# joshua16266261/self-play-ai

Measured on AMD Instinct MI355X. Metric: MCTS sims/sec + self-play games/sec, Connect4 800 sims/move, 1/2/4/8 GPU, higher is better.
Workload: dtype bf16

## Files before the change

self-play-ai_amd/csrc/search.hip:

```cpp
#include <algorithm>
#include <cstdlib>
#include <cstring>

#include "search_internal.h"

namespace spai {
namespace {

constexpr int kLanesPerTree = 8;
#ifndef SPAI_TREE_BLOCK
#define SPAI_TREE_BLOCK 64
#endif
constexpr int kBlock = SPAI_TREE_BLOCK;
constexpr int kTreesPerBlock = kBlock / kLanesPerTree;
constexpr uint32_t kErrNan = 1u, kErrCapacity = 2u, kErrDepth = 4u;

constexpr uint32_t kPriorMark = 0x80000000u;
constexpr int kGenShift = 49;

__device__ __forceinline__ float ucb(float sqrt_np, const uint4 &ch, float c) {
    const uint32_t n = ch.x;
    const float w = __uint_as_float(ch.y), prior = __uint_as_float(ch.z);
    const float qv = ((-w / (float)(n == 0 ? 1u : n)) + 1.0f) / 2.0f;
    const float q = n == 0 ? 0.0f : qv;
    float u = c * prior;
    u = u * sqrt_np;
    u = u / (1.0f + (float)n);
    return q + u;
}

constexpr int kLevelsPerLane = kMaxDepth / kLanesPerTree;
__device__ __forceinline__ void backup_load(const uint4 *nodes, const uint32_t (&node)[kLevelsPerLane], int d,
                                            int lane8, uint2 (&r)[kLevelsPerLane]) {
#pragma unroll
    for (int j = 0; j < kLevelsPerLane; ++j) r[j] = *(const uint2 *)(nodes + (lane8 + 8 * j <= d ? node[j] : node[0]));
}
__device__ __forceinline__ void backup_store(uint4 *nodes, const uint32_t (&node)[kLevelsPerLane], int d, float v,
                                             int lane8, const uint2 (&r)[kLevelsPerLane]) {
#pragma unroll
    for (int j = 0; j < kLevelsPerLane; ++j) {
        const int lvl = lane8 + 8 * j;
        if (lvl <= d) {
            const float sign = ((d - lvl) & 1) ? -1.0f : 1.0f;
            *(uint2 *)(nodes + node[j]) = make_uint2(r[j].x + 1u, __float_as_uint(__uint_as_float(r[j].y) + sign * v));
        }
    }
}
__device__ __forceinline__ void backup_nodes(uint4 *nodes, const uint32_t (&node)[kLevelsPerLane], int d, float v,
                                             int lane8) {
    uint2 r[kLevelsPerLane];
    backup_load(nodes, node, d, lane8, r);
    backup_store(nodes, node, d, v, lane8, r);
}

__device__ __forceinline__ uint32_t group_bits(uint64_t ball) {
    return (uint32_t)(ball >> (threadIdx.x & 63 & ~(kLanesPerTree - 1))) & 0xFFu;
}

__device__ __forceinline__ bool has_line_flat(uint64_t b) {
    const uint64_t h = b & (b >> 7), v = b & (b >> 1), g = b & (b >> 8);
    return ((h & (h >> 14)) | (v & (v >> 2)) | (g & (g >> 16))) != 0ull;
}

__device__ __forceinline__ uint32_t score_key(float u) {
    const uint32_t b = __float_as_uint(u + 0.0f);
    return (b & 0x80000000u) ? ~b : (b | 0x80000000u);
}

struct Cand {
    uint32_t hi, lo, n, w;
};
template <int CTRL>
__device__ __forceinline__ uint32_t dpp_mov(uint32_t v) {
    return (uint32_t)__builtin_amdgcn_mov_dpp((int)v, CTRL, 0xF, 0xF, true);
}
template <int CTRL>
__device__ __forceinline__ void cand_step(Cand &c) {
    const Cand o{dpp_mov<CTRL>(c.hi), dpp_mov<CTRL>(c.lo), dpp_mov<CTRL>(c.n), dpp_mov<CTRL>(c.w)};
    const bool take = (((uint64_t)o.hi << 32) | o.lo) > (((uint64_t)c.hi << 32) | c.lo);
    c.hi = take ? o.hi : c.hi;
    c.lo = take ? o.lo : c.lo;
    c.n = take ? o.n : c.n;
    c.w = take ? o.w : c.w;
}

struct RootInfo {
    uint32_t node;
    uint64_t x, o;
    uint8_t n, status;
    uint32_t rn, rw;
};
__device__ __forceinline__ RootInfo load_root(const TreeView &T, uint32_t t) {
    const uint32_t node = T.root[t];
    const uint4 r = T.nodes[(size_t)t * T.cap + node];
    return RootInfo{node, T.root_x[t], T.root_o[t], T.root_n[t], T.root_status[t], r.x, r.w};
}

enum Descent { kTerminal = 0, kLive = 1, kError = 2 };
__device__ __forceinline__ Descent descend(const TreeView &T, uint32_t t, const RootInfo &root, int lane8, float c,
                                           uint32_t *err, uint64_t &x, uint64_t &o, uint8_t &n) {
    uint4 *nodes = T.nodes + (size_t)t * T.cap;
    uint32_t *path = T.path + (size_t)t * kMaxDepth;
    uint32_t node = root.node;
    x = root.x;
    o = root.o;
    n = root.n;
    uint8_t status = root.status;
    uint32_t rn = root.rn, rw = root.rw;
    uint32_t pr[kLevelsPerLane] = {node, 0u, 0u, 0u, 0u, 0u};
    const int top = 7 * lane8 + 5;
    int d = 0;
    if (lane8 == 0) path[0] = node;
    while (rw != kNoChildren) {
        const uint32_t first = rw & 0xFFFFFFu;
        const uint64_t occ = x | o;
        const bool open = lane8 < c4::kActions && !((occ >> top) & 1ull);
        const uint32_t k = c4::popc32(group_bits(__ballot(open)) & ((1u << lane8) - 1u));
        const uint4 ch = nodes[first + (open ? k : 0u)];
        const float sq = sqrtf((float)rn);
        const float u = ucb(sq, ch, c);
        Cand w{open ? score_key(u) : 0u, ((uint32_t)lane8 << 3) | k, ch.x, ch.w};
        cand_step<0xB1>(w);
        cand_step<0x4E>(w);
        cand_step<0x141>(w);
        if (group_bits(__ballot(open && u != u))) {
            if (lane8 == 0) atomicOr(err, kErrNan);
            return kError;
        }
        rn = w.n;
        rw = w.w;
        const int a = (int)(w.lo >> 3);
        const uint64_t bit = c4::drop_bit(occ, a);
        const bool xm = c4::x_to_move(n);
        x = xm ? x | bit : x;
        o = xm ? o : o | bit;
        n = (uint8_t)(n + 1);
        status = has_line_flat(xm ? x : o) ? c4::kWon : (n == c4::kCells ? c4::kTied : c4::kOngoing);
        node = first + (w.lo & 7u);
        ++d;
        if (d >= kMaxDepth) {
            if (lane8 == 0) atomicOr(err, kErrDepth);
            return kError;
        }
        const bool mine = (d & 7) == lane8;
        if (mine) path[d] = node;
#pragma unroll
        for (int j = 0; j < kLevelsPerLane; ++j) pr[j] = mine && (d >> 3) == j ? node : pr[j];
    }
    if (lane8 == 0) T.depth[t] = (uint8_t)d;
    if (status != c4::kOngoing) {
        backup_nodes(nodes, pr, d, c4::terminal_value(status), lane8);
        return kTerminal;
    }
    return kLive;
}

__device__ __forceinline__ uint4 *cache_way(const CacheView &C, uint64_t mine, uint64_t theirs, int way) {
    const uint64_t h = c4::splitmix64(mine ^ (theirs * 0x9E3779B97F4A7C15ull));
    const uint32_t bucket = (uint32_t)(h >> 32) & C.mask;
    return C.tab + ((size_t)bucket * EvalCache::kWays + (uint32_t)way) * 4;
}

__device__ __forceinline__ bool cache_insert(const CacheView &C, const BatchView &B, uint32_t s, int lane8) {
    const uint64_t mine = B.mine[s], theirs = B.theirs[s];
    const uint64_t gen = (uint64_t)C.gen << kGenShift;
    const uint64_t k0 = mine | gen, k1 = theirs | gen;
    uint4 *bucket = cache_way(C, mine, theirs, 0);
    const uint64_t seen = *(const uint64_t *)(bucket + 4 * lane8);
    const float4 pa = *(const float4 *)(B.priors + (size_t)s * kPriorStride);
    const float4 pb = *(const float4 *)(B.priors + (size_t)s * kPriorStride + 4);
    const float value = B.value[s];
    const uint32_t same = group_bits(__ballot(seen == k0));
    const uint32_t empty = group_bits(__ballot(seen == 0ull));
    if (same || lane8 != 0) return false;
    const uint32_t p0 = __float_as_uint(pa.x), p2 = __float_as_uint(pa.z), p4 = __float_as_uint(pb.x),
                   p6 = __float_as_uint(pb.z);
    bool claimed = false, skip = ((p0 | p2 | p4 | p6) & kPriorMark) != 0u;
    if (!skip)
        for (int w = empty ? __ffs(empty) - 1 : (int)EvalCache::kWays; w < (int)EvalCache::kWays; ++w) {
            uint4 *e = bucket + 4 * w;
            const unsigned long long old = atomicCAS((unsigned long long *)e, 0ull, (unsigned long long)k0);
            if (old == 0ull) {
                ((uint64_t *)e)[1] = k1;
                e[1] = make_uint4(p0 | kPriorMark, __float_as_uint(pa.y), p2 | kPriorMark, __float_as_uint(pa.w));
                e[2] = make_uint4(p4 | kPriorMark, __float_as_uint(pb.y), p6 | kPriorMark, __float_as_uint(value));
                claimed = true;
                break;
            }
            if (old == k0) {
                skip = true;
                break;
            }
        }
    if (!claimed && !skip) atomicAdd(C.ctr + 1, 1u);
    return claimed;
}
__device__ __forceinline__ void cache_count(const CacheView &C, bool claimed) {
    const uint64_t b = __ballot(claimed);
    if (b && (threadIdx.x & 63) == (uint32_t)__ffsll((unsigned long long)__ballot(true)) - 1u)
        atomicAdd(C.ctr, (uint32_t)c4::popc64(b));
}

__device__ __forceinline__ void slot_leaf(const TreeView &T, const BatchView &B, const CacheView &C, uint32_t t,
                                          int lane8, uint64_t x, uint64_t o, uint8_t n) {
    const bool xm = c4::x_to_move(n);
    const uint64_t mine = xm ? x : o, theirs = xm ? o : x;
    if (lane8 == 0)
        __hip_atomic_fetch_add(T.evals + t, 1u, __ATOMIC_RELAXED, __HIP_MEMORY_SCOPE_AGENT);
    if (C.tab) {
        const uint4 *e = cache_way(C, mine, theirs, lane8);
        const uint4 q0 = e[0], q1 = e[1], q2 = e[2];
        const uint64_t gen = (uint64_t)C.gen << kGenShift;
        const bool match = (((uint64_t)q0.y << 32) | q0.x) == (mine | gen) &&
                           (((uint64_t)q0.w << 32) | q0.z) == (theirs | gen) &&
                           (q1.x & q1.z & q2.x & q2.z & kPriorMark) != 0u;
        const uint32_t hit = group_bits(__ballot(match));
        if (hit) {
            uint32_t slot = 0;
            if (lane8 == 0) {
                slot = B.cap - 1u - atomicAdd(B.hits, 1u);
                T.slot[t] = slot | kHitSlot;
                B.tree[slot] = t;
                B.mine[slot] = mine;
                B.theirs[slot] = theirs;
            }
            slot = (uint32_t)__shfl((int)slot, 0, kLanesPerTree);
            if (lane8 == __ffs(hit) - 1) {
                float4 *pr = (float4 *)(B.priors + (size_t)slot * kPriorStride);
                pr[0] = make_float4(__uint_as_float(q1.x & ~kPriorMark), __uint_as_float(q1.y),
                                    __uint_as_float(q1.z & ~kPriorMark), __uint_as_float(q1.w));
                pr[1] = make_float4(__uint_as_float(q2.x & ~kPriorMark), __uint_as_float(q2.y),
                                    __uint_as_float(q2.z & ~kPriorMark), 0.f);
                B.value[slot] = __uint_as_float(q2.w);
            }
            return;
        }
    }
    if (lane8 == 0) {
        const uint32_t slot = atomicAdd(B.count, 1u);
        T.slot[t] = slot;
        B.tree[slot] = t;
        B.mine[slot] = mine;
        B.theirs[slot] = theirs;
    }
}

template <bool RUN_ON>
__device__ __forceinline__ void select_tree(const TreeView &T, const BatchView &B, const CacheView &C, uint32_t t,
                                            RootInfo &root, int lane8, float c, uint32_t *err, uint32_t run_cap) {
    if (lane8 == 0) T.slot[t] = kNoSlot;
    uint64_t x, o;
    uint8_t n;
    if (!RUN_ON) {
        if (descend(T, t, root, lane8, c, err, x, o, n) == kLive) slot_leaf(T, B, C, t, lane8, x, o, n);
        return;
    }
    uint32_t left = T.left[t];
    for (uint32_t run = 0; left > 0; ++run) {
        if (run == run_cap) {
            if (lane8 == 0) atomicOr(B.more, 1u);
            break;
        }
        --left;
        const Descent r = descend(T, t, root, lane8, c, err, x, o, n);
        if (r == kLive) slot_leaf(T, B, C, t, lane8, x, o, n);
        if (r != kTerminal) break;
        root.rn += 1;
        __builtin_amdgcn_fence(__ATOMIC_SEQ_CST, "wavefront");
    }
    if (lane8 == 0) T.left[t] = left;
}

struct LeafPath {
    int d;
    uint32_t lv[kLevelsPerLane];
    uint32_t first;
};
__device__ __forceinline__ LeafPath load_leaf_path(const TreeView &T, uint32_t t, int lane8) {
    LeafPath L;
    const uint32_t *path = T.path + (size_t)t * kMaxDepth;
    L.d = T.depth[t];
#pragma unroll
    for (int j = 0; j < kLevelsPerLane; ++j) L.lv[j] = path[lane8 + 8 * j];
    L.first = T.next_free[t];
    return L;
}

__device__ __forceinline__ void expand_leaf(const TreeView &T, const BatchView &B, uint32_t t, uint32_t s, int lane8,
                                            uint32_t *err, const LeafPath &L, RootInfo &root) {
    uint4 *nodes = T.nodes + (size_t)t * T.cap;
    const int d = L.d;
    uint32_t node[kLevelsPerLane];
#pragma unroll
    for (int j = 0; j < kLevelsPerLane; ++j) node[j] = lane8 + 8 * j <= d ? L.lv[j] : 0u;
    const uint64_t occ = B.mine[s] | B.theirs[s];
    const float prior = B.priors[(size_t)s * kPriorStride + lane8];
    const float value = B.value[s];
    uint2 r[kLevelsPerLane];
    backup_load(nodes, node, d, lane8, r);
    const bool legal = lane8 < c4::kActions && !((occ >> (7 * lane8 + 5)) & 1ull);
    const uint32_t grp = group_bits(__ballot(legal));
    const uint32_t nch = c4::popc32(grp);
    const uint32_t idx = c4::popc32(grp & ((1u << lane8) - 1u));
    const uint32_t first = L.first;
    if (first + nch > T.cap) {
        if (lane8 == 0) atomicOr(err, kErrCapacity);
        return;
    }
    if (legal) nodes[first + idx] = make_uint4(0u, 0u, __float_as_uint(prior), kNoChildren);
    if (lane8 == 0) T.next_free[t] = first + nch;
    if (lane8 == (d & 7)) {
        uint32_t leaf = node[0];
#pragma unroll
        for (int j = 1; j < kLevelsPerLane; ++j) leaf = (d >> 3) == j ? node[j] : leaf;
        nodes[leaf].w = first | (nch << 24);
    }
    backup_store(nodes, node, d, value, lane8, r);
    root.rn += 1;
    if (d == 0) root.rw = first | (nch << 24);
}

template <bool RUN_ON>
__global__ __launch_bounds__(kBlock) void k_select(TreeView T, BatchView B, CacheView C,
                                                   const uint32_t *__restrict__ active, uint32_t n_active, float c,
                                                   uint32_t *err, uint32_t run_cap) {
    const uint32_t gi = (blockIdx.x * blockDim.x + threadIdx.x) / kLanesPerTree;
#ifdef SPAI_TREE_PRIO
    __builtin_amdgcn_s_setprio(SPAI_TREE_PRIO);
#endif
    if (gi >= n_active) return;
    const uint32_t t = active[gi];
    RootInfo root = load_root(T, t);
    select_tree<RUN_ON>(T, B, C, t, root, threadIdx.x & (kLanesPerTree - 1), c, err, run_cap);
}

template <bool RUN_ON>
__global__ __launch_bounds__(kBlock) void k_expand_select(TreeView T, BatchView cur, BatchView nxt, CacheView C,
                                                          const uint32_t *__restrict__ active, uint32_t n_active,
                                                          float c, uint32_t *err, uint32_t run_cap) {
    const uint32_t gi = (blockIdx.x * blockDim.x + threadIdx.x) / kLanesPerTree;
#ifdef SPAI_TREE_PRIO
    __builtin_amdgcn_s_setprio(SPAI_TREE_PRIO);
#endif
    if (gi >= n_active) return;
    const int lane8 = threadIdx.x & (kLanesPerTree - 1);
    const uint32_t t = active[gi];
    const uint32_t s = T.slot[t];
    RootInfo root = load_root(T, t);
    const LeafPath L = load_leaf_path(T, t, lane8);
    asm volatile("" ::"v"(root.rn), "v"(root.rw), "v"((uint32_t)root.x), "v"((uint32_t)(root.x >> 32)),
                 "v"((uint32_t)root.o), "v"((uint32_t)(root.o >> 32)), "v"((uint32_t)root.n), "v"((uint32_t)root.status));
    asm volatile("" ::"v"(L.d), "v"(L.first), "v"(L.lv[0]), "v"(L.lv[1]), "v"(L.lv[2]), "v"(L.lv[3]), "v"(L.lv[4]),
                 "v"(L.lv[5]));
    if (s != kNoSlot) expand_leaf(T, cur, t, s & ~kHitSlot, lane8, err, L, root);
    __builtin_amdgcn_fence(__ATOMIC_SEQ_CST, "wavefront");
    select_tree<RUN_ON>(T, nxt, C, t, root, lane8, c, err, run_cap);
    if (C.tab) {
        const bool claimed = s != kNoSlot && !(s & kHitSlot) && cache_insert(C, cur, s, lane8);
        cache_count(C, claimed);
    }
}

__global__ void k_set_left(TreeView T, const uint32_t *__restrict__ active, uint32_t n, uint32_t iters) {
    const uint32_t i = blockIdx.x * blockDim.x + threadIdx.x;
    if (i < n) T.left[active[i]] = iters;
}

__global__ __launch_bounds__(kBlock) void k_eval_stub(BatchView B, uint32_t max_n, int kind) {
    const uint32_t s = blockIdx.x * blockDim.x + threadIdx.x;
    if (s >= max_n || s >= *B.count) return;
    const uint32_t n = (uint32_t)c4::popc64(B.mine[s] | B.theirs[s]);
    const bool xm = (n & 1u) == 0;
    const uint64_t x = xm ? B.mine[s] : B.theirs[s], o = xm ? B.theirs[s] : B.mine[s];
    float pr[c4::kActions], v;
    c4::stub_eval(kind, x, o, (uint8_t)n, pr, &v);
    for (int a = 0; a < c4::kActions; ++a) B.priors[(size_t)s * kPriorStride + a] = pr[a];
    B.value[s] = v;
}

__global__ __launch_bounds__(kBlock) void k_expand(TreeView T, BatchView B, CacheView C, uint32_t max_n,
                                                   uint32_t *err) {
    const uint32_t i = (blockIdx.x * blockDim.x + threadIdx.x) / kLanesPerTree;
    if (i >= max_n) return;
    const uint32_t count = *B.count, hits = B.hits ? *B.hits : 0u;
    if (i >= count + hits) return;
    const bool fwd = i < count;
    const uint32_t s = fwd ? i : B.cap - 1u - (i - count);
    const int lane8 = threadIdx.x & (kLanesPerTree - 1);
    const uint32_t t = B.tree[s];
    RootInfo root{};
    expand_leaf(T, B, t, s, lane8, err, load_leaf_path(T, t, lane8), root);
    if (C.tab) {
        const bool claimed = fwd && cache_insert(C, B, s, lane8);
        cache_count(C, claimed);
    }
}

__global__ void k_root_stats(TreeView T, const uint32_t *__restrict__ active, uint32_t n_active, uint32_t *out,
                             uint32_t *max_evals) {
    const uint32_t i = blockIdx.x * blockDim.x + threadIdx.x;
    if (i >= n_active) return;
    const uint32_t t = active[i];
    atomicMax(max_evals, T.evals[t]);
    atomicAdd(max_evals + 1, T.evals[t]);
    const uint4 *nodes = T.nodes + (size_t)t * T.cap;
    const uint4 r = nodes[T.root[t]];
    out[i * 8] = r.w;
    const uint32_t nch = r.w == kNoChildren ? 0 : r.w >> 24, first = r.w & 0xFFFFFFu;
    for (uint32_t k = 0; k < 7; ++k) out[i * 8 + 1 + k] = k < nch ? nodes[first + k].x : 0u;
}

__global__ void k_trees_init(TreeView T, RootsOut R, uint32_t first_tree, uint32_t n) {
    const uint32_t i = blockIdx.x * blockDim.x + threadIdx.x;
    if (i < n) tree_clear(T, R, first_tree + i);
}
}

TreeView tree_view(spai_engine *e) {
    Trees &T = e->trees;
    return TreeView{T.nodes.p, T.cap, T.root.p, T.next_free.p, T.root_x.p, T.root_o.p, T.root_n.p, T.root_status.p,
                    T.path.p, T.depth.p, T.slot.p, T.left.p, T.evals.p};
}

static BatchView batch_view(spai_engine *e, int chain, uint32_t it, bool cached) {
    Batch &B = e->batch[chain];
    const size_t h = (size_t)(it & 1u) * B.cap;
    return BatchView{B.iter_counts.p + it, B.iter_more.p ? B.iter_more.p + it : nullptr, B.tree.p + h, B.mine.p + h, B.theirs.p + h,
                     B.priors.p + h * kPriorStride, B.value.p + h,
                     cached ? B.iter_hits.p + it : nullptr, B.cap};
}

CacheView cache_view(spai_engine *e) {
    EvalCache &C = e->cache;
    if (!C.buckets) return CacheView{nullptr, 0u, 0u, nullptr};
    return CacheView{C.table.p, C.buckets - 1u, C.gen, C.ctr.p};
}

int cache_clear(spai_engine *e) {
    EvalCache &C = e->cache;
    if (!C.buckets) return SPAI_OK;
    uint32_t fill = 0;
    SPAI_HIP(hipMemcpyAsync(&fill, C.ctr.p, 4, hipMemcpyDeviceToHost, e->stream));
    SPAI_HIP(hipStreamSynchronize(e->stream));
    C.inserts_cleared += fill;
    SPAI_HIP(hipMemsetAsync(C.table.p, 0, C.table.n * sizeof(uint4), e->stream));
    SPAI_HIP(hipMemsetAsync(C.ctr.p, 0, 4, e->stream));
    C.gen = C.gen % 32767u + 1u;
    C.fill_seen = 0;
    C.clears += 1;
    return SPAI_OK;
}

int cache_prepare(spai_engine *e, bool for_net) {
    EvalCache &C = e->cache;
    if (C.ready && C.for_net == for_net) return SPAI_OK;
    C.for_net = for_net;
    uint64_t want = 0;
    if (for_net) {
        const char *v = std::getenv("SPAI_EVAL_CACHE");
        if (C.user_set) want = C.requested;
        else if (v) want = std::strtoull(v, nullptr, 10);
        else want = std::min<uint64_t>(EvalCache::kEntriesPerTree * std::max(1u, e->cfg.max_trees),
                                       EvalCache::kDefaultMaxEntries);
    }
    uint32_t buckets = 0;
    if (want) {
        buckets = 1;
        while ((uint64_t)buckets * 2 * EvalCache::kWays <= want && buckets < (1u << 28)) buckets *= 2;
    }
    if (buckets != C.buckets) {
        SPAI_HIP(hipStreamSynchronize(e->stream));
        if (C.buckets) {
            uint32_t fill = 0;
            SPAI_HIP(hipMemcpy(&fill, C.ctr.p, 4, hipMemcpyDeviceToHost));
            C.inserts_cleared += fill;
        }
        C.buckets = 0;
        if (C.ctr.p) SPAI_HIP(hipMemsetAsync(C.ctr.p, 0, 4, e->stream));
        const bool by_default = !C.user_set && !std::getenv("SPAI_EVAL_CACHE");
        int rc = C.table.alloc((size_t)buckets * EvalCache::kWays * 4);
        while (rc != SPAI_OK && by_default) {
            (void)hipGetLastError();
            buckets = buckets / 2 >= EvalCache::kMinDefaultBuckets ? buckets / 2 : 0;
            rc = C.table.alloc((size_t)buckets * EvalCache::kWays * 4);
        }
        SPAI_TRY(rc);
        if (buckets) {
            if (!C.ctr.p) {
                SPAI_TRY(C.ctr.alloc(2));
                SPAI_HIP(hipMemsetAsync(C.ctr.p, 0, 8, e->stream));
            }
            C.buckets = buckets;
            SPAI_TRY(cache_clear(e));
        }
    }
    C.ready = true;
    return SPAI_OK;
}

constexpr double kMinChainLeaves = 64;
constexpr double kTailLeaves = 0.05;
constexpr uint32_t kTailTreeEvals = 160;
constexpr uint32_t kTailRun = 128;
static int env_int(const char *name, int dflt) {
    const char *v = std::getenv(name);
    return v ? std::atoi(v) : dflt;
}
struct ChainPolicy {
    int chains;
    uint32_t grid_cap;
};
static ChainPolicy chains_for(uint32_t n, double last_evals_per_iter) {
    static const int forced = std::max(0, std::min(spai_engine::kChains, env_int("SPAI_CHAINS", 0)));
    static const int mid_leaves = env_int("SPAI_MID_LEAVES", 0);
    static const int mid_chains = std::max(1, std::min(spai_engine::kChains, env_int("SPAI_MID_CHAINS", 2)));
    static const uint32_t mid_grid = (uint32_t)std::max(0, env_int("SPAI_MID_GRID", 0));
    static const double min_chain_leaves = env_int("SPAI_MIN_CHAIN_LEAVES", (int)kMinChainLeaves);
    static const int hi_leaves = env_int("SPAI_HI_LEAVES", 0);
    if (forced) return {std::max(1, std::min<int>(forced, (int)(n / 64))), 0u};
    if (hi_leaves > 0 && (last_evals_per_iter < 0 ? (double)n : last_evals_per_iter) >= hi_leaves) return {1, 0u};
    if (last_evals_per_iter >= 0 && last_evals_per_iter < min_chain_leaves) return {1, 0u};
    if (last_evals_per_iter >= 0 && last_evals_per_iter < mid_leaves)
        return {std::max(1, std::min<int>(mid_chains, (int)(n / 64))), mid_grid};
    return {std::max(1, std::min<int>(2, (int)(n / 64))), 0u};
}

static int upload_roots(spai_engine *e, uint32_t t0, uint32_t n) {
    Trees &T = e->trees;
    std::vector<uint64_t> x(n), o(n);
    std::vector<uint8_t> nn(n), st(n);
    for (uint32_t i = 0; i < n; ++i) {
        const c4::State &s = T.h_root_state[t0 + i];
        x[i] = s.x;
        o[i] = s.o;
        nn[i] = s.n;
        st[i] = s.status;
    }
    hipStream_t s = e->stream;
    SPAI_HIP(hipMemcpyAsync(T.root.p + t0, T.h_root.data() + t0, n * 4, hipMemcpyHostToDevice, s));
    SPAI_HIP(hipMemcpyAsync(T.root_x.p + t0, x.data(), n * 8, hipMemcpyHostToDevice, s));
    SPAI_HIP(hipMemcpyAsync(T.root_o.p + t0, o.data(), n * 8, hipMemcpyHostToDevice, s));
    SPAI_HIP(hipMemcpyAsync(T.root_n.p + t0, nn.data(), n, hipMemcpyHostToDevice, s));
    SPAI_HIP(hipMemcpyAsync(T.root_status.p + t0, st.data(), n, hipMemcpyHostToDevice, s));
    SPAI_HIP(hipStreamSynchronize(s));
    return SPAI_OK;
}

static int timer_record(spai_engine *e, int which, uint32_t iter, bool begin, hipStream_t st, int chain) {
    KernelTimer &K = e->timer;
    if (!K.enabled) return SPAI_OK;
    if (begin) {
        if (K.used + 2 > K.ev.size()) {
            for (int i = 0; i < 64; ++i) {
                hipEvent_t ev;
                SPAI_HIP(hipEventCreate(&ev));
                K.ev.push_back(ev);
            }
        }
        K.which.push_back(which);
        K.iter.push_back(iter);
        K.chain.push_back(chain);
        SPAI_HIP(hipEventRecord(K.ev[K.used], st));
    } else {
        SPAI_HIP(hipEventRecord(K.ev[K.used + 1], st));
        K.used += 2;
    }
    return SPAI_OK;
}

static int timer_collect(spai_engine *e, const uint32_t *ch_counts, uint32_t num_searches, const Chain *chains) {
    KernelTimer &K = e->timer;
    if (!K.enabled) return SPAI_OK;
    for (size_t i = 0; i < K.which.size(); ++i) {
        float ms = 0;
        SPAI_HIP(hipEventElapsedTime(&ms, K.ev[2 * i], K.ev[2 * i + 1]));
        const int w = K.which[i], h = K.chain[i];
        K.total_ms[w] += ms;
        K.launches[w] += 1;
        K.items[w] += w == 0 ? chains[h].cnt : ch_counts[(size_t)h * num_searches + K.iter[i]];
    }
    K.used = 0;
    K.which.clear();
    K.iter.clear();
    K.chain.clear();
    return SPAI_OK;
}

int trees_create(spai_engine *e, uint32_t n) {
    SPAI_CHECK(n > 0 && n <= e->cfg.max_trees, SPAI_ERR_INVALID, "trees_create: n=%u exceeds max_trees=%u", n,
               e->cfg.max_trees);
    Trees &T = e->trees;
    const uint64_t cap = 1ull + (uint64_t)c4::kActions * e->cfg.num_searches * std::max(1u, e->cfg.max_moves);
    SPAI_CHECK(cap < (1ull << 24), SPAI_ERR_CAPACITY, "node arena of %llu nodes per tree exceeds 2^24",
               (unsigned long long)cap);
    if (T.n_trees != n || T.cap != cap) {
        T.n_trees = 0;
        SPAI_TRY(T.nodes.alloc((size_t)n * cap));
        SPAI_TRY(T.root.alloc(n));
        SPAI_TRY(T.next_free.alloc(n));
        SPAI_TRY(T.root_x.alloc(n));
        SPAI_TRY(T.root_o.alloc(n));
        SPAI_TRY(T.root_n.alloc(n));
        SPAI_TRY(T.root_status.alloc(n));
        SPAI_TRY(T.path.alloc((size_t)n * kMaxDepth));
        SPAI_TRY(T.depth.alloc(n));
        SPAI_TRY(T.slot.alloc(n));
        SPAI_TRY(T.left.alloc(n));
        SPAI_TRY(T.evals.alloc(n + 2));
        SPAI_TRY(T.slot_gid.alloc(n));
        SPAI_TRY(T.slot_move.alloc(n));
        SPAI_TRY(T.refill.alloc(2 * (size_t)n));
        SPAI_TRY(e->active.alloc(n));
        SPAI_TRY(e->stats.alloc((size_t)n * 8));
        for (Batch &B : e->batch) {
            SPAI_TRY(B.tree.alloc(2 * (size_t)n));
            SPAI_TRY(B.mine.alloc(2 * (size_t)n));
            SPAI_TRY(B.theirs.alloc(2 * (size_t)n));
            SPAI_TRY(B.priors.alloc(2 * (size_t)n * kPriorStride));
            SPAI_TRY(B.value.alloc(2 * (size_t)n));
            B.cap = n;
        }
        T.n_trees = n;
        T.cap = (uint32_t)cap;
    }
    e->last_evals_per_iter = -1;
    e->last_served_per_iter = -1;
    e->last_max_tree_evals = ~0u;
    T.h_root.assign(n, 0);
    T.h_root_state.assign(n, c4::State{0, 0, 0, c4::kOngoing});
    T.h_root_first.assign(n, 0);
    T.h_root_nch.assign(n, 0);
    k_trees_init<<<(n + 255) / 256, 256, 0, e->stream>>>(tree_view(e), roots_out(e), 0, n);
    SPAI_HIP(hipGetLastError());
    return upload_roots(e, 0, n);
}

int tree_reset(spai_engine *e, uint32_t t, const spai_c4_state *root) {
    Trees &T = e->trees;
    SPAI_CHECK(t < T.n_trees, SPAI_ERR_INVALID, "tree %u out of range", t);
    c4::State s{0, 0, 0, c4::kOngoing};
    if (root) {
        SPAI_CHECK(!(root->x & root->o) && !((root->x | root->o) & ~c4::kBoard) && root->status <= c4::kWon,
                   SPAI_ERR_INVALID, "root is not a Connect4 bitboard");
        s = from_abi(*root);
    }
    T.h_root[t] = 0;
    T.h_root_state[t] = s;
    T.h_root_first[t] = 0;
    T.h_root_nch[t] = 0;
    k_trees_init<<<1, 64, 0, e->stream>>>(tree_view(e), roots_out(e), t, 1);
    SPAI_HIP(hipGetLastError());
    return upload_roots(e, t, 1);
}

static int evaluate(const Chain &c, hipStream_t st, const BatchView &bv, uint32_t grid_cap, int conc) {
    if (c.kind == SPAI_EVAL_NET)
        return net_eval_batch(c.net, st, bv.count, c.cnt, bv.mine, bv.theirs, bv.priors, bv.value, grid_cap, conc);
    k_eval_stub<<<(c.cnt + kBlock - 1) / kBlock, kBlock, 0, st>>>(bv, c.cnt, c.kind);
    return SPAI_OK;
}

int chains_launch(spai_engine *e, const uint32_t *trees, const Chain *chains, int nchain, uint32_t grid_cap, bool timed,
                  bool tail) {
    hipStream_t st = e->stream;
    uint32_t n = 0, iters = 0;
    int conc = 0;
    for (int h = 0; h < nchain; ++h) {
        const Chain &c = chains[h];
        if (!c.cnt) continue;
        n += c.cnt;
        iters = std::max(iters, c.iters);
        conc += c.kind == SPAI_EVAL_NET;
        Batch &B = e->batch[h];
        const uint32_t nc = std::max<uint32_t>(c.iters, 1) + (tail ? kTailChunk + 1 : 0);
        DevBuf<uint32_t> *ctr[3] = {&B.iter_counts, c.cache.tab ? &B.iter_hits : nullptr,
                                    tail ? &B.iter_more : nullptr};
        for (DevBuf<uint32_t> *b : ctr) {
            if (!b) continue;
            if (b->n < nc) SPAI_TRY(b->alloc(nc));
            SPAI_HIP(hipMemsetAsync(b->p, 0, (size_t)nc * 4, st));
        }
    }
    SPAI_HIP(hipMemcpyAsync(e->active.p, trees, (size_t)n * 4, hipMemcpyHostToDevice, st));
    SPAI_HIP(hipMemsetAsync(e->err.p, 0, 4, st));
    SPAI_HIP(hipMemsetAsync(e->trees.evals.p, 0, ((size_t)e->trees.n_trees + 2) * 4, st));
    if (n > chains[0].cnt) SPAI_HIP(hipEventRecord(e->ev_fork, st));
    for (int h = 1; h < nchain; ++h)
        if (chains[h].cnt) SPAI_HIP(hipStreamWaitEvent(e->chain_stream[h], e->ev_fork, 0));
    const TreeView tv = tree_view(e);
    timed = timed && e->timer.enabled;
    for (uint32_t it = 0; it < (tail ? 0u : iters); ++it) {
        for (int h = 0; h < nchain; ++h) {
            const Chain &c = chains[h];
            if (!c.cnt || it >= c.iters) continue;
            const hipStream_t sh = e->chain_stream[h];
            const BatchView bv = batch_view(e, h, it, c.cache.tab);
            const uint32_t nh = c.cnt, g8 = (nh + kTreesPerBlock - 1) / kTreesPerBlock;
            const uint32_t *act = e->active.p + c.off;
            const bool sample = timed && (it % e->timer.stride == 0);
            if (it == 0) {
                if (sample) SPAI_TRY(timer_record(e, 0, it, true, sh, h));
                k_select<false><<<g8, kBlock, 0, sh>>>(tv, bv, c.cache, act, nh, e->cfg.c, e->err.p, 0u);
                if (sample) SPAI_TRY(timer_record(e, 0, it, false, sh, h));
            }
            if (sample) SPAI_TRY(timer_record(e, 1, it, true, sh, h));
            SPAI_TRY(evaluate(c, sh, bv, grid_cap, std::max(conc, 1)));
            if (sample) SPAI_TRY(timer_record(e, 1, it, false, sh, h));
            if (it + 1 < c.iters) {
                const bool s2 = timed && ((it + 1) % e->timer.stride == 0);
                if (s2) SPAI_TRY(timer_record(e, 0, it + 1, true, sh, h));
                k_expand_select<false><<<g8, kBlock, 0, sh>>>(tv, bv, batch_view(e, h, it + 1, c.cache.tab), c.cache,
                                                              act, nh, e->cfg.c, e->err.p, 0u);
                if (s2) SPAI_TRY(timer_record(e, 0, it + 1, false, sh, h));
            } else {
                if (sample) SPAI_TRY(timer_record(e, 2, it, true, sh, h));
                k_expand<<<g8, kBlock, 0, sh>>>(tv, bv, c.cache, nh, e->err.p);
                if (sample) SPAI_TRY(timer_record(e, 2, it, false, sh, h));
            }
        }
    }
    SPAI_HIP(hipGetLastError());
    for (int h = 1; h < nchain; ++h) {
        if (!chains[h].cnt) continue;
        SPAI_HIP(hipEventRecord(e->ev_join[h], e->chain_stream[h]));
        SPAI_HIP(hipStreamWaitEvent(st, e->ev_join[h], 0));
    }
    return SPAI_OK;
}

int search_launch(spai_engine *e, uint32_t n, const uint32_t *tree_idx, uint32_t num_searches, SearchRun &R) {
    const int kind = (int)e->cfg.eval;
    hipStream_t st = e->stream;
    SPAI_TRY(cache_prepare(e, kind == SPAI_EVAL_NET));
    if (cache_nearly_full(e->cache)) SPAI_TRY(cache_clear(e));
    const char *tl_env = std::getenv("SPAI_TAIL_LEAVES");
    const char *tt_env = std::getenv("SPAI_TAIL_TREE_EVALS");
    const double tail_leaves = tl_env ? std::atof(tl_env) : kTailLeaves;
    const uint32_t tail_tree = tt_env ? (uint32_t)std::max(0, std::atoi(tt_env)) : kTailTreeEvals;
    const bool tail = num_searches > 0 && e->last_served_per_iter >= 0 &&
                      (e->last_served_per_iter < tail_leaves || e->last_max_tree_evals < tail_tree);
    const bool solved = e->last_served_per_iter == 0.0;
    const char *tr_env = std::getenv("SPAI_TAIL_RUN");
    const uint32_t tail_run =
        tr_env ? (uint32_t)std::max(1, std::atoi(tr_env)) : (solved ? std::max(num_searches, 1u) : kTailRun);
    const uint32_t tail_chunk = solved ? 1u : kTailChunk;
    const ChainPolicy pol = tail ? ChainPolicy{1, 0u} : chains_for(n, e->last_evals_per_iter);
    const int nchain = R.nchain = pol.chains;
    const CacheView cv = cache_view(e);
    for (int h = 0; h < nchain; ++h) {
        const uint32_t off = (uint32_t)((uint64_t)n * h / nchain);
        R.chain[h] = Chain{off, (uint32_t)((uint64_t)n * (h + 1) / nchain) - off, num_searches, kind, e->net, cv};
    }
    SPAI_TRY(chains_launch(e, tree_idx, R.chain, nchain, pol.grid_cap, true, tail));
    R.n_counts = num_searches;
    if (tail) {
        const TreeView tv = tree_view(e);
        const uint32_t g8 = (n + kTreesPerBlock - 1) / kTreesPerBlock;
        const uint32_t *act = e->active.p;
        k_set_left<<<(n + 255) / 256, 256, 0, st>>>(tv, act, n, num_searches);
        k_select<true><<<g8, kBlock, 0, st>>>(tv, batch_view(e, 0, 0, cv.tab), cv, act, n, e->cfg.c, e->err.p, tail_run);
        uint32_t p = 0, next = 1, more = 0, next_hits = 0;
        for (;;) {
            for (uint32_t q = 0; q < tail_chunk; ++q, ++p) {
                const BatchView bv = batch_view(e, 0, p, cv.tab);
                SPAI_TRY(evaluate(R.chain[0], st, bv, 0u, 1));
                k_expand_select<true><<<g8, kBlock, 0, st>>>(tv, bv, batch_view(e, 0, p + 1, cv.tab), cv, act, n,
                                                             e->cfg.c, e->err.p, tail_run);
            }
            SPAI_HIP(hipGetLastError());
            SPAI_HIP(hipMemcpyAsync(&next, e->batch[0].iter_counts.p + p, 4, hipMemcpyDeviceToHost, st));
            SPAI_HIP(hipMemcpyAsync(&more, e->batch[0].iter_more.p + p, 4, hipMemcpyDeviceToHost, st));
            if (cv.tab)
                SPAI_HIP(hipMemcpyAsync(&next_hits, e->batch[0].iter_hits.p + p, 4, hipMemcpyDeviceToHost, st));
            SPAI_HIP(hipStreamSynchronize(st));
            next += next_hits;
            if (next == 0 && more == 0) break;
            SPAI_CHECK(p <= num_searches + 1, SPAI_ERR_INVALID, "internal: tail passes exceed the iterations");
        }
        R.n_counts = p;
    }
    e->last_tail_passes = tail ? R.n_counts : 0;
    return SPAI_OK;
}

int check_device_errors(spai_engine *e, uint32_t err) {
    SPAI_CHECK(!(err & kErrCapacity), SPAI_ERR_CAPACITY, "node arena full (cap %u per tree)", e->trees.cap);
    SPAI_CHECK(!(err & kErrDepth), SPAI_ERR_CAPACITY, "tree deeper than %d", kMaxDepth);
    SPAI_CHECK(!(err & kErrNan), SPAI_ERR_NAN, "NaN UCB in select (reference: partial_cmp().unwrap() panics)");
    return SPAI_OK;
}

void cache_account(spai_engine *e, double served, double forwarded, uint32_t fill) {
    if (!e->cache.buckets) return;
    e->cache.lookups += served;
    e->cache.hits += served - forwarded;
    e->cache.fill_seen = fill;
}

int search_finish(spai_engine *e, const SearchRun &R, uint32_t num_searches, const uint32_t *ch_counts, uint32_t err,
                  uint32_t max_tree_evals, double served, uint32_t cache_fill) {
    SPAI_TRY(timer_collect(e, ch_counts, R.n_counts, R.chain));
    double s = 0;
    for (int h = 0; h < R.nchain; ++h)
        for (uint32_t i = 0; i < R.n_counts; ++i) s += ch_counts[(size_t)h * R.n_counts + i];
    SPAI_TRY(check_device_errors(e, err));
    cache_account(e, served, s, cache_fill);
    e->last_evals_per_iter = num_searches ? s / num_searches : -1;
    e->last_served_per_iter = num_searches ? served / num_searches : -1;
    e->last_max_tree_evals = max_tree_evals;
    return SPAI_OK;
}

int search(spai_engine *e, uint32_t n, const uint32_t *tree_idx, uint32_t num_searches, float *policy,
           uint32_t *child_ids, float *child_visits, uint32_t *n_children, double *evals_out) {
    Trees &T = e->trees;
    SPAI_CHECK(T.n_trees > 0, SPAI_ERR_INVALID, "no trees: call spai_trees_create first");
    SPAI_CHECK(n <= T.n_trees, SPAI_ERR_INVALID, "search over %u trees, %u exist", n, T.n_trees);
    for (uint32_t i = 0; i < n; ++i) SPAI_CHECK(tree_idx[i] < T.n_trees, SPAI_ERR_INVALID, "tree %u out of range", tree_idx[i]);
    const int kind = (int)e->cfg.eval;
    SPAI_CHECK(kind != SPAI_EVAL_NET || e->net, SPAI_ERR_INVALID, "eval = NET but no net set (spai_engine_set_net)");
    if (n == 0) return SPAI_OK;
    hipStream_t st = e->stream;
    SearchRun R;
    SPAI_TRY(search_launch(e, n, tree_idx, num_searches, R));
    const TreeView tv = tree_view(e);
    const int nchain = R.nchain;
    const uint32_t n_counts = R.n_counts;
    k_root_stats<<<(n + 255) / 256, 256, 0, st>>>(tv, e->active.p, n, e->stats.p, T.evals.p + T.n_trees);
    SPAI_HIP(hipGetLastError());
    std::vector<uint32_t> stats((size_t)n * 8), ch_counts((size_t)nchain * n_counts);
    uint32_t err = 0, tree_evals[2] = {0, 0}, cache_fill = 0;
    SPAI_HIP(hipMemcpyAsync(stats.data(), e->stats.p, stats.size() * 4, hipMemcpyDeviceToHost, st));
    SPAI_HIP(hipMemcpyAsync(tree_evals, T.evals.p + T.n_trees, 8, hipMemcpyDeviceToHost, st));
    if (e->cache.buckets) SPAI_HIP(hipMemcpyAsync(&cache_fill, e->cache.ctr.p, 4, hipMemcpyDeviceToHost, st));
    if (n_counts)
        for (int h = 0; h < nchain; ++h)
            SPAI_HIP(hipMemcpyAsync(ch_counts.data() + (size_t)h * n_counts, e->batch[h].iter_counts.p,
                                    n_counts * 4, hipMemcpyDeviceToHost, st));
    SPAI_HIP(hipMemcpyAsync(&err, e->err.p, 4, hipMemcpyDeviceToHost, st));
    SPAI_HIP(hipStreamSynchronize(st));
    SPAI_TRY(search_finish(e, R, num_searches, ch_counts.data(), err, tree_evals[0], tree_evals[1], cache_fill));
    if (evals_out) *evals_out = (double)tree_evals[1];
    for (uint32_t i = 0; i < n; ++i) {
        const uint32_t t = tree_idx[i];
        const uint32_t w = stats[i * 8];
        const uint32_t nch = w == kNoChildren ? 0 : w >> 24, first = w & 0xFFFFFFu;
        T.h_root_first[t] = first;
        T.h_root_nch[t] = (uint8_t)nch;
        const c4::State &rs = T.h_root_state[t];
        const uint32_t legal = c4::legal_mask(rs.x, rs.o, rs.status);
        float pol[c4::kActions] = {0, 0, 0, 0, 0, 0, 0};
        for (uint32_t k = 0; k < nch; ++k) {
            const float v = (float)stats[i * 8 + 1 + k];
            pol[c4::kth_bit(legal, (int)k)] = v;
            if (child_ids) child_ids[(size_t)i * 7 + k] = first + k;
            if (child_visits) child_visits[(size_t)i * 7 + k] = v;
        }
        for (uint32_t k = nch; k < 7; ++k) {
            if (child_ids) child_ids[(size_t)i * 7 + k] = kNoChildren;
            if (child_visits) child_visits[(size_t)i * 7 + k] = 0.f;
        }
        if (n_children) n_children[i] = nch;
        if (policy) normalize_policy(pol, policy + (size_t)i * 7);
    }
    return SPAI_OK;
}

int tree_use_subtree(spai_engine *e, uint32_t t, uint32_t child) {
    Trees &T = e->trees;
    SPAI_CHECK(t < T.n_trees, SPAI_ERR_INVALID, "tree %u out of range", t);
    const uint32_t first = T.h_root_first[t], nch = T.h_root_nch[t];
    SPAI_CHECK(nch > 0 && child >= first && child < first + nch, SPAI_ERR_INVALID,
               "node %u is not a child of tree %u's root (run spai_search first)", child, t);
    const c4::State &rs = T.h_root_state[t];
    c4::State ns;
    const int a = c4::kth_bit(c4::legal_mask(rs.x, rs.o, rs.status), (int)(child - first));
    SPAI_CHECK(c4::next_state(rs, a, ns) == 0, SPAI_ERR_INVALID, "internal: root child replay failed");
    T.h_root[t] = child;
    T.h_root_state[t] = ns;
    T.h_root_nch[t] = 0;
    return upload_roots(e, t, 1);
}

int tree_node(spai_engine *e, uint32_t t, uint32_t node, spai_c4_state *st, uint32_t *visits, float *w) {
    Trees &T = e->trees;
    SPAI_CHECK(t < T.n_trees, SPAI_ERR_INVALID, "tree %u out of range", t);
    c4::State s = T.h_root_state[t];
    if (node != T.h_root[t]) {
        const uint32_t first = T.h_root_first[t], nch = T.h_root_nch[t];
        SPAI_CHECK(nch > 0 && node >= first && node < first + nch, SPAI_ERR_INVALID,
                   "node %u: only the root and its children are addressable", node);
        const int a = c4::kth_bit(c4::legal_mask(s.x, s.o, s.status), (int)(node - first));
        c4::State ns;
        c4::next_state(s, a, ns);
        s = ns;
    }
    if (st) *st = to_abi(s);
    if (visits || w) {
        uint4 rec;
        SPAI_HIP(hipMemcpy(&rec, T.nodes.p + (size_t)t * T.cap + node, 16, hipMemcpyDeviceToHost));
        if (visits) *visits = rec.x;
        if (w) memcpy(w, &rec.y, 4);
    }
    return SPAI_OK;
}

int tree_size(spai_engine *e, uint32_t t, uint32_t *nodes) {
    Trees &T = e->trees;
    SPAI_CHECK(t < T.n_trees, SPAI_ERR_INVALID, "tree %u out of range", t);
    SPAI_HIP(hipMemcpy(nodes, T.next_free.p + t, 4, hipMemcpyDeviceToHost));
    return SPAI_OK;
}


int eval_cache_set_capacity(spai_engine *e, uint64_t entries) {
    e->cache.user_set = true;
    e->cache.requested = entries;
    e->cache.ready = false;
    return SPAI_OK;
}

int eval_cache_clear(spai_engine *e) { return cache_clear(e); }

int eval_cache_stats(spai_engine *e, spai_eval_cache_stats *out) {
    EvalCache &C = e->cache;
    uint32_t ctr[2] = {0, 0};
    SPAI_HIP(hipStreamSynchronize(e->stream));
    if (C.ctr.p) SPAI_HIP(hipMemcpy(ctr, C.ctr.p, 8, hipMemcpyDeviceToHost));
    out->lookups = C.lookups;
    out->hits = C.hits;
    out->inserts = C.inserts_cleared + ctr[0];
    out->dropped = ctr[1];
    out->clears = C.clears;
    out->capacity = (double)C.entries();
    return SPAI_OK;
}

}
```

Before: 70.01 million.

## Aggregate leaf slot atomics per wavefront and overlap cache insert probe with selection

```diff
diff --git a/self-play-ai_amd/csrc/search.hip b/self-play-ai_amd/csrc/search.hip
--- a/self-play-ai_amd/csrc/search.hip
+++ b/self-play-ai_amd/csrc/search.hip
@@ -161,17 +161,32 @@
     return C.tab + ((size_t)bucket * EvalCache::kWays + (uint32_t)way) * 4;
 }
 
-__device__ __forceinline__ bool cache_insert(const CacheView &C, const BatchView &B, uint32_t s, int lane8) {
-    const uint64_t mine = B.mine[s], theirs = B.theirs[s];
+struct InsertProbe {
+    uint64_t k0, k1, seen;
+    uint4 *bucket;
+    float4 pa, pb;
+    float value;
+};
+__device__ __forceinline__ InsertProbe insert_probe(const CacheView &C, const BatchView &B, uint32_t s, uint64_t mine,
+                                                    uint64_t theirs, int lane8) {
+    InsertProbe P;
     const uint64_t gen = (uint64_t)C.gen << kGenShift;
-    const uint64_t k0 = mine | gen, k1 = theirs | gen;
-    uint4 *bucket = cache_way(C, mine, theirs, 0);
-    const uint64_t seen = *(const uint64_t *)(bucket + 4 * lane8);
-    const float4 pa = *(const float4 *)(B.priors + (size_t)s * kPriorStride);
-    const float4 pb = *(const float4 *)(B.priors + (size_t)s * kPriorStride + 4);
-    const float value = B.value[s];
-    const uint32_t same = group_bits(__ballot(seen == k0));
-    const uint32_t empty = group_bits(__ballot(seen == 0ull));
+    P.k0 = mine | gen;
+    P.k1 = theirs | gen;
+    P.bucket = cache_way(C, mine, theirs, 0);
+    P.seen = *(const uint64_t *)(P.bucket + 4 * lane8);
+    P.pa = *(const float4 *)(B.priors + (size_t)s * kPriorStride);
+    P.pb = *(const float4 *)(B.priors + (size_t)s * kPriorStride + 4);
+    P.value = B.value[s];
+    return P;
+}
+__device__ __forceinline__ bool insert_claim(const CacheView &C, const InsertProbe &P, int lane8) {
+    const uint64_t k0 = P.k0, k1 = P.k1;
+    uint4 *bucket = P.bucket;
+    const float4 pa = P.pa, pb = P.pb;
+    const float value = P.value;
+    const uint32_t same = group_bits(__ballot(P.seen == k0));
+    const uint32_t empty = group_bits(__ballot(P.seen == 0ull));
     if (same || lane8 != 0) return false;
     const uint32_t p0 = __float_as_uint(pa.x), p2 = __float_as_uint(pa.z), p4 = __float_as_uint(pb.x),
                    p6 = __float_as_uint(pb.z);
@@ -207,41 +222,44 @@
     const uint64_t mine = xm ? x : o, theirs = xm ? o : x;
     if (lane8 == 0)
         __hip_atomic_fetch_add(T.evals + t, 1u, __ATOMIC_RELAXED, __HIP_MEMORY_SCOPE_AGENT);
+    uint32_t hit = 0;
+    uint4 q1 = make_uint4(0u, 0u, 0u, 0u), q2 = q1;
     if (C.tab) {
         const uint4 *e = cache_way(C, mine, theirs, lane8);
-        const uint4 q0 = e[0], q1 = e[1], q2 = e[2];
+        const uint4 q0 = e[0];
+        q1 = e[1];
+        q2 = e[2];
         const uint64_t gen = (uint64_t)C.gen << kGenShift;
         const bool match = (((uint64_t)q0.y << 32) | q0.x) == (mine | gen) &&
                            (((uint64_t)q0.w << 32) | q0.z) == (theirs | gen) &&
                            (q1.x & q1.z & q2.x & q2.z & kPriorMark) != 0u;
-        const uint32_t hit = group_bits(__ballot(match));
-        if (hit) {
-            uint32_t slot = 0;
-            if (lane8 == 0) {
-                slot = B.cap - 1u - atomicAdd(B.hits, 1u);
-                T.slot[t] = slot | kHitSlot;
-                B.tree[slot] = t;
-                B.mine[slot] = mine;
-                B.theirs[slot] = theirs;
-            }
-            slot = (uint32_t)__shfl((int)slot, 0, kLanesPerTree);
-            if (lane8 == __ffs(hit) - 1) {
-                float4 *pr = (float4 *)(B.priors + (size_t)slot * kPriorStride);
-                pr[0] = make_float4(__uint_as_float(q1.x & ~kPriorMark), __uint_as_float(q1.y),
-                                    __uint_as_float(q1.z & ~kPriorMark), __uint_as_float(q1.w));
-                pr[1] = make_float4(__uint_as_float(q2.x & ~kPriorMark), __uint_as_float(q2.y),
-                                    __uint_as_float(q2.z & ~kPriorMark), 0.f);
-                B.value[slot] = __uint_as_float(q2.w);
-            }
-            return;
-        }
-    }
+        hit = group_bits(__ballot(match));
+    }
+    const uint32_t lane = threadIdx.x & 63u;
+    const uint64_t hitb = __ballot(lane8 == 0 && hit), missb = __ballot(lane8 == 0 && !hit);
+    const uint32_t hl = hitb ? (uint32_t)__ffsll((unsigned long long)hitb) - 1u : 64u;
+    const uint32_t ml = missb ? (uint32_t)__ffsll((unsigned long long)missb) - 1u : 64u;
+    uint32_t base = 0;
+    if (lane == hl || lane == ml)
+        base = atomicAdd(lane == hl ? B.hits : B.count, (uint32_t)c4::popc64(lane == hl ? hitb : missb));
+    const uint32_t hbase = (uint32_t)__builtin_amdgcn_readlane((int)base, (int)(hl & 63u));
+    const uint32_t mbase = (uint32_t)__builtin_amdgcn_readlane((int)base, (int)(ml & 63u));
+    const uint64_t below = (1ull << (lane & ~(uint32_t)(kLanesPerTree - 1))) - 1ull;
+    const uint32_t rank = (uint32_t)c4::popc64((hit ? hitb : missb) & below);
+    const uint32_t slot = hit ? B.cap - 1u - (hbase + rank) : mbase + rank;
     if (lane8 == 0) {
-        const uint32_t slot = atomicAdd(B.count, 1u);
-        T.slot[t] = slot;
+        T.slot[t] = hit ? slot | kHitSlot : slot;
         B.tree[slot] = t;
         B.mine[slot] = mine;
         B.theirs[slot] = theirs;
+    }
+    if (hit && lane8 == __ffs(hit) - 1) {
+        float4 *pr = (float4 *)(B.priors + (size_t)slot * kPriorStride);
+        pr[0] = make_float4(__uint_as_float(q1.x & ~kPriorMark), __uint_as_float(q1.y),
+                            __uint_as_float(q1.z & ~kPriorMark), __uint_as_float(q1.w));
+        pr[1] = make_float4(__uint_as_float(q2.x & ~kPriorMark), __uint_as_float(q2.y),
+                            __uint_as_float(q2.z & ~kPriorMark), 0.f);
+        B.value[slot] = __uint_as_float(q2.w);
     }
 }
 
@@ -287,13 +305,16 @@
 }
 
 __device__ __forceinline__ void expand_leaf(const TreeView &T, const BatchView &B, uint32_t t, uint32_t s, int lane8,
-                                            uint32_t *err, const LeafPath &L, RootInfo &root) {
+                                            uint32_t *err, const LeafPath &L, RootInfo &root, uint64_t &mine,
+                                            uint64_t &theirs) {
     uint4 *nodes = T.nodes + (size_t)t * T.cap;
     const int d = L.d;
     uint32_t node[kLevelsPerLane];
 #pragma unroll
     for (int j = 0; j < kLevelsPerLane; ++j) node[j] = lane8 + 8 * j <= d ? L.lv[j] : 0u;
-    const uint64_t occ = B.mine[s] | B.theirs[s];
+    mine = B.mine[s];
+    theirs = B.theirs[s];
+    const uint64_t occ = mine | theirs;
     const float prior = B.priors[(size_t)s * kPriorStride + lane8];
     const float value = B.value[s];
     uint2 r[kLevelsPerLane];
@@ -352,13 +373,17 @@
                  "v"((uint32_t)root.o), "v"((uint32_t)(root.o >> 32)), "v"((uint32_t)root.n), "v"((uint32_t)root.status));
     asm volatile("" ::"v"(L.d), "v"(L.first), "v"(L.lv[0]), "v"(L.lv[1]), "v"(L.lv[2]), "v"(L.lv[3]), "v"(L.lv[4]),
                  "v"(L.lv[5]));
-    if (s != kNoSlot) expand_leaf(T, cur, t, s & ~kHitSlot, lane8, err, L, root);
+    const bool ins = C.tab && s != kNoSlot && !(s & kHitSlot);
+    InsertProbe P{};
+    uint64_t mine = 0, theirs = 0;
+    if (s != kNoSlot) {
+        expand_leaf(T, cur, t, s & ~kHitSlot, lane8, err, L, root, mine, theirs);
+        if (ins) P = insert_probe(C, cur, s, mine, theirs, lane8);
+    }
     __builtin_amdgcn_fence(__ATOMIC_SEQ_CST, "wavefront");
     select_tree<RUN_ON>(T, nxt, C, t, root, lane8, c, err, run_cap);
-    if (C.tab) {
-        const bool claimed = s != kNoSlot && !(s & kHitSlot) && cache_insert(C, cur, s, lane8);
-        cache_count(C, claimed);
-    }
+    const bool claimed = ins && insert_claim(C, P, lane8);
+    if (C.tab) cache_count(C, claimed);
 }
 
 __global__ void k_set_left(TreeView T, const uint32_t *__restrict__ active, uint32_t n, uint32_t iters) {
@@ -389,9 +414,10 @@
     const int lane8 = threadIdx.x & (kLanesPerTree - 1);
     const uint32_t t = B.tree[s];
     RootInfo root{};
-    expand_leaf(T, B, t, s, lane8, err, load_leaf_path(T, t, lane8), root);
+    uint64_t mine, theirs;
+    expand_leaf(T, B, t, s, lane8, err, load_leaf_path(T, t, lane8), root, mine, theirs);
     if (C.tab) {
-        const bool claimed = fwd && cache_insert(C, B, s, lane8);
+        const bool claimed = fwd && insert_claim(C, insert_probe(C, B, s, mine, theirs, lane8), lane8);
         cache_count(C, claimed);
     }
 }
@@ -511,7 +537,7 @@
     uint32_t grid_cap;
 };
 static ChainPolicy chains_for(uint32_t n, double last_evals_per_iter) {
-    static const int forced = std::max(0, std::min(spai_engine::kChains, env_int("SPAI_CHAINS", 0)));
+    const int forced = std::max(0, std::min(spai_engine::kChains, env_int("SPAI_CHAINS", 0)));
     static const int mid_leaves = env_int("SPAI_MID_LEAVES", 0);
     static const int mid_chains = std::max(1, std::min(spai_engine::kChains, env_int("SPAI_MID_CHAINS", 2)));
     static const uint32_t mid_grid = (uint32_t)std::max(0, env_int("SPAI_MID_GRID", 0));
```

New measurement: 70.48 million (median of 6 runs). No clear change (+0.7%).
